# Fabri000/Maze-Solving-Agent-Gymnasium

Hardware: AMD Instinct MI355X
Metric: env steps/sec (whole node) + DQN win-rate, 40x40 r-prim mazes (higher is better)
Workload: dtype int32

## Files before the change

include/mazerl.h:

```cpp
#ifndef MAZERL_H
#define MAZERL_H
#include <stdint.h>

#ifdef __cplusplus
extern "C" {
#endif

#define MZ_OK 0
#define MZ_EINVAL (-1)
#define MZ_EINVAL_SHAPE (-2)
#define MZ_EHIP (-3)
#define MZ_ENOMEM (-4)
#define MZ_EALIGN (-5)

#define MZ_MAX_DIM 127
#define MZ_BANK_MAX_DIMS 64
#define MZ_MAX_CANDIDATES 64
#define MZ_WINDOW 15
#define MZ_WINDOW_BITS 675
#define MZ_WINDOW_WORDS 22

#define MZ_ALGO_RPRIM 0
#define MZ_ALGO_DFS 1
#define MZ_ALGO_PRIMKILL 2
// ... 58 lines not shown
int mz_generate_state(mz_handle* h, int32_t env, int32_t dim, int32_t algo, uint32_t* state_host,
                      void* stream);

int mz_reset_all(mz_handle* h, const mz_step_out* out, void* stream);
int mz_reset_list(mz_handle* h, const int32_t* idx_dev, const int32_t* count_dev,
                  int32_t max_count, int32_t regen_won, uint64_t seed, uint32_t epoch,
                  const mz_step_out* out, void* stream);

int mz_reset_done(mz_handle* h, int32_t regen_won, uint64_t seed, uint32_t epoch,
                  const mz_step_out* out, void* stream);

int mz_step(mz_handle* h, const int32_t* actions_dev, const mz_step_out* out, void* stream);

#define MZ_STEP_COUNT_ZEROED 1
#define MZ_STEP_AUTORESET 2
int mz_step_ex(mz_handle* h, const int32_t* actions_dev, const mz_step_out* out, int32_t flags,
               void* stream);

int mz_step_act(mz_handle* h, const float* eps_dev, float eps_all, const int64_t* greedy_dev,
                uint64_t seed, uint64_t counter, int32_t* actions_out_dev, const mz_step_out* out,
                int32_t flags, void* stream);

int mz_direction_mask(mz_handle* h, int32_t probs, float* out4_dev, void* stream);

int mz_act(mz_handle* h, const float* eps_dev, float eps_all, const int64_t* greedy_dev,
           uint64_t seed, uint64_t counter, int32_t* actions_dev, void* stream);

int mz_expand_window(const uint32_t* bits_dev, float* out_dev, int32_t n, void* stream);

int mz_bank_create(mz_handle* h, int32_t slots, int32_t dim, uint32_t algo_mask);
// ... 226 lines not shown
```

maze-solving-agent-gymnasium_amd/csrc/mz_api.hip:

```cpp
#include <algorithm>
#include <cmath>
#include <cstdarg>
#include <cstdio>
#include <cstdlib>
#include <cstring>
#include <string>
#include <vector>

#include "../../include/mazerl.h"
#include "mz_common.h"
#include "mz_learner.h"
#include "mz_mcclendon.h"

struct MzHostFallback {
  int cap = 0, gstride = 0;
  uint8_t *grid_h = nullptr, *grid_d = nullptr;
  int32_t *info_h = nullptr, *info_d = nullptr;
  double *prod_h = nullptr, *prod_d = nullptr;
  int32_t *ok_h = nullptr, *ok_d = nullptr;
  int32_t* count_h = nullptr;
  int* count_d = nullptr;
  int32_t* map = nullptr;
};

// ... 30 lines not shown
};

struct mz_handle {
  mz_config cfg;
  MzDev d;
  std::vector<void*> allocs;
  uint8_t* staging = nullptr;
  size_t staging_bytes = 0;
  MzBankStore bank;
  MzCandStore gen;
  int* sel_stats = nullptr;
  int dbg = 0;
  std::vector<void*> host_allocs;
  MzCompact scr{};
  int scr_cap = 0;
};

namespace {

thread_local std::string g_err;

int fail(int code, const char* fmt, ...) {
  char buf[512];
  va_list ap;
  va_start(ap, fmt);
  vsnprintf(buf, sizeof buf, fmt, ap);
  va_end(ap);
  g_err = buf;
  return code;
}
// ... 34 lines not shown
  MzOut m;
  std::memset(&m, 0, sizeof m);
  if (!o) return m;
  m.reward = o->reward; m.reward64 = o->reward64; m.terminated = o->terminated;
  m.truncated = o->truncated; m.pos = o->pos; m.best_dir = o->best_dir; m.obs6 = o->obs6;
  m.window_bits = o->window_bits; m.window = o->window; m.done_idx = o->done_idx;
  m.done_count = o->done_count;
  return m;
}

int check_out(const mz_step_out* o) {
  if (o && o->window && (reinterpret_cast<uintptr_t>(o->window) & 15u))
    return fail(MZ_EALIGN, "window output must be 16-byte aligned");
  if (o && o->done_idx && !o->done_count) return fail(MZ_EINVAL, "done_idx needs done_count");
  return MZ_OK;
}

int check_dim(const mz_handle* h, int dim) {
  if (dim < 5 || dim > h->cfg.max_dim)
    return fail(MZ_EINVAL_SHAPE, "maze dim %d outside [5, max_dim=%d]", dim, h->cfg.max_dim);
  if ((dim & 1) == 0)
    return fail(MZ_EINVAL_SHAPE, "even maze dim %d (reference gen_maze raises IndexError, "
                "lib/maze_generation.py:197-203)", dim);
  if (h->cfg.enrich && !h->cfg.toroidal && dim < 15)
    return fail(MZ_EINVAL_SHAPE, "euclidean window needs dim >= 15 (extract_submaze, "
                "lib/maze_handler.py:18-45)");
  return MZ_OK;
}

template <typename T>
// ... 310 lines not shown

int mz_reset_done(mz_handle* h, int32_t regen_won, uint64_t seed, uint32_t epoch,
                  const mz_step_out* out, void* stream) {
  if (!h) return fail(MZ_EINVAL, "null handle");
  int rc = check_out(out);
  if (rc) return rc;
  DeviceGuard g(h->cfg.device);
  MZ_HIP(mz_launch_reset_done(h->d, regen_won ? 1 : 0, seed, epoch, to_dev(out),
                              static_cast<hipStream_t>(stream)));
  return MZ_OK;
}

int mz_step_ex(mz_handle* h, const int32_t* actions_dev, const mz_step_out* out, int32_t flags,
               void* stream) {
  if (!h || !actions_dev) return fail(MZ_EINVAL, "bad arguments");
  if (flags & ~(MZ_STEP_COUNT_ZEROED | MZ_STEP_AUTORESET)) return fail(MZ_EINVAL, "flags %d", flags);
  int rc = check_out(out);
  if (rc) return rc;
  DeviceGuard g(h->cfg.device);
  hipStream_t s = static_cast<hipStream_t>(stream);
  if (out && out->done_count && !(flags & MZ_STEP_COUNT_ZEROED))
    MZ_HIP(hipMemsetAsync(out->done_count, 0, sizeof(int32_t), s));
  MZ_HIP(mz_launch_step(h->d, actions_dev, nullptr, (flags & MZ_STEP_AUTORESET) != 0, to_dev(out), s));
  return MZ_OK;
}

int mz_step(mz_handle* h, const int32_t* actions_dev, const mz_step_out* out, void* stream) {
  return mz_step_ex(h, actions_dev, out, 0, stream);
}

int mz_step_act(mz_handle* h, const float* eps_dev, float eps_all, const int64_t* greedy_dev,
                uint64_t seed, uint64_t counter, int32_t* actions_out_dev, const mz_step_out* out,
                int32_t flags, void* stream) {
  if (!h) return fail(MZ_EINVAL, "null handle");
  if (flags & ~(MZ_STEP_COUNT_ZEROED | MZ_STEP_AUTORESET)) return fail(MZ_EINVAL, "flags %d", flags);
  int rc = check_out(out);
  if (rc) return rc;
  DeviceGuard g(h->cfg.device);
  hipStream_t s = static_cast<hipStream_t>(stream);
  if (out && out->done_count && !(flags & MZ_STEP_COUNT_ZEROED))
    MZ_HIP(hipMemsetAsync(out->done_count, 0, sizeof(int32_t), s));
  MzAct ap{eps_dev, eps_all, greedy_dev, seed, counter, actions_out_dev};
  MZ_HIP(mz_launch_step(h->d, nullptr, &ap, (flags & MZ_STEP_AUTORESET) != 0, to_dev(out), s));
  return MZ_OK;
}

int mz_direction_mask(mz_handle* h, int32_t probs, float* out4_dev, void* stream) {
  if (!h || !out4_dev) return fail(MZ_EINVAL, "bad arguments");
  if (reinterpret_cast<uintptr_t>(out4_dev) & 15u) return fail(MZ_EALIGN, "out4 must be 16-B aligned");
  DeviceGuard g(h->cfg.device);
  MZ_HIP(mz_launch_mask(h->d, probs, out4_dev, static_cast<hipStream_t>(stream)));
  return MZ_OK;
}

int mz_act(mz_handle* h, const float* eps_dev, float eps_all, const int64_t* greedy_dev,
           uint64_t seed, uint64_t counter, int32_t* actions_dev, void* stream) {
  if (!h || !actions_dev) return fail(MZ_EINVAL, "bad arguments");
  DeviceGuard g(h->cfg.device);
// ... 513 lines not shown
  bool same_bank = hdr[SH_BK_K] == (uint32_t)b.K && hdr[SH_BK_NA] == (uint32_t)b.nA &&
                   hdr[SH_BK_ND] == (uint32_t)b.nD && hdr[SH_BK_AMASK] == b.amask;
  for (int i = 0; same_bank && i < b.nD; ++i) same_bank = dims[i] == (uint8_t)b.dims[i];
  if (!same_bank)
    return fail(MZ_EINVAL, "env state has a maze bank of %u slots x %u algorithms x %u sizes "
                "(mask %u); this handle's is %d x %d x %d (mask %u)", hdr[SH_BK_K], hdr[SH_BK_NA],
                hdr[SH_BK_ND], hdr[SH_BK_AMASK], b.K, b.nA, b.nD, b.amask);
  if (bytes < state_size(h)) return fail(MZ_EINVAL, "state buffer of %llu bytes, %zu needed",
                                         (unsigned long long)bytes, state_size(h));
  const uint8_t* src = static_cast<const uint8_t*>(src_dev);
  size_t off = MZ_STATE_HEADER_BYTES;
  for (const Section& sec : state_sections(h)) {
    MZ_HIP(hipMemcpyAsync(sec.p, src + off, sec.bytes, hipMemcpyDeviceToDevice, s));
    off += (sec.bytes + 255) & ~(size_t)255;
  }
  if (b.K) {
    b.epoch[0] = hdr[SH_BK_EPOCH0];
    b.epoch[1] = hdr[SH_BK_EPOCH1];
  }
  return mz_bank_use(h, (int32_t)hdr[SH_BK_ACTIVE]);
}

int mz_maze_metrics(mz_handle* h, const int32_t* env_ids_dev, int32_t n, double* out_dev,
                    void* stream) {
  if (!h || !out_dev) return fail(MZ_EINVAL, "bad arguments");
  if (h->d.toroidal) return fail(MZ_EINVAL, "maze metrics are defined for euclidean mazes");
  if (!env_ids_dev) n = h->d.B;
  if (n < 0 || n > h->d.B) return fail(MZ_EINVAL, "n out of range");
  DeviceGuard g(h->cfg.device);
  MZ_HIP(mz_launch_metrics(h->d, env_ids_dev, n, out_dev, static_cast<hipStream_t>(stream)));
// ... 555 lines not shown
```

maze-solving-agent-gymnasium_amd/csrc/mz_common.h:

```cpp
#pragma once
#include <hip/hip_runtime.h>
#include <stdint.h>

#define MZ_CELL_D_MASK 0x1FFFu
#define MZ_CELL_CODE_SHIFT 13
#define MZ_CELL_OPEN (1u << 16)
#define MZ_CELL_NB_SHIFT 17
#define MZ_CELL_CNT_SHIFT 21
#define MZ_CELL_TAG_SHIFT 29
#define MZ_CELL_STATIC ((1u << MZ_CELL_CNT_SHIFT) - 1u)
#define MZ_STW_TAG_SHIFT 24

__host__ __device__ inline int mz_cell_count(uint32_t w, uint32_t tag) {
  return (w >> MZ_CELL_TAG_SHIFT) == tag ? (int)((w >> MZ_CELL_CNT_SHIFT) & 0xFFu) : 0;
}
#define MZ_TICKET_PYERR 8

struct MzDev {
  int B, P, toroidal, enrich;
  int NS, PW;
  uint32_t* cells;
  uint32_t* planes;
  uint32_t* meta0;
  uint32_t* meta1;
  uint32_t* posw;
  uint32_t* stw;
// ... 37 lines not shown
};

struct MzOut {
  float* reward;
  double* reward64;
  uint8_t* terminated;
  uint8_t* truncated;
  int32_t* pos;
  int32_t* best_dir;
  float* obs6;
  uint32_t* window_bits;
  float* window;
  int32_t* done_idx;
  int32_t* done_count;
  int window_nt;
};
#define MZ_WINDOW_NT_BYTES (256ull << 20)

__host__ __device__ inline int mz_dr(int a) { return a == 0 ? 1 : (a == 1 ? -1 : 0); }
__host__ __device__ inline int mz_dc(int a) { return a == 2 ? 1 : (a == 3 ? -1 : 0); }
__host__ __device__ inline int mz_wrap(int v, int n) { v %= n; return v < 0 ? v + n : v; }
__host__ __device__ inline int mz_wrapn(int v, int n) {
  while (v < 0) v += n;
  while (v >= n) v -= n;
  return v;
}

__host__ __device__ inline void mz_philox(uint64_t key, uint64_t ctr_hi, uint64_t ctr_lo,
                                          uint32_t out[4]) {
  uint32_t c0 = (uint32_t)ctr_lo, c1 = (uint32_t)(ctr_lo >> 32), c2 = (uint32_t)ctr_hi,
// ... 59 lines not shown
```

maze-solving-agent-gymnasium_amd/csrc/mz_env.hip:

```cpp
#include "mz_common.h"
#include "mz_kernels.h"
#include "mz_build.inc.h"

#include "../../include/mazerl.h"

#define WAVE 64
#ifndef MZ_IPW
#define MZ_IPW 16
#endif
#define IPW MZ_IPW
#ifndef MZ_SPW
#define MZ_SPW 1
#endif
#ifndef MZ_PROBE
#define MZ_PROBE 0
#endif
__host__ __device__ constexpr int cat_words(int ipw) { return ipw * 675 / 32 + 2; }

namespace {

__device__ inline uint32_t wrap_colmask(int col, int C0, int N) {
  uint32_t m = 0;
  for (int j = mz_wrapn(col - C0, N); j < 15; j += N) m |= 1u << j;
  return m;
}

template <bool TOR>
__device__ inline int win_geo(int r, int c, int N) {
  int R0, C0;
  if (!TOR) { R0 = mz_win_start(r, N); C0 = mz_win_start(c, N); }
// ... 74 lines not shown
__device__ inline void write_obs6(float* o6, int r, int c, int gr, int gc, int br, int bc, int N) {
  if (ENRICH) {
    const double n = (double)N;
    o6[0] = (float)__ddiv_rn((double)r, n);
    o6[1] = (float)__ddiv_rn((double)c, n);
    o6[2] = (float)__ddiv_rn((double)gr, n);
    o6[3] = (float)__ddiv_rn((double)gc, n);
  } else {
    o6[0] = (float)r; o6[1] = (float)c; o6[2] = (float)gr; o6[3] = (float)gc;
  }
  o6[4] = (float)br;
  o6[5] = (float)bc;
}

typedef __attribute__((ext_vector_type(4))) unsigned int mz_u32x4;
template <int POL = 16>
__device__ inline void store_window_f32(const uint32_t* cat, float* out, int nb, int lane) {
  const int nfl = nb * 675;
  const int nq = nfl >> 2;
  const auto rsrc = __builtin_amdgcn_make_buffer_rsrc(out, 0, nfl * 4, 0x00020000);
  auto put = [&](int q, uint32_t word) {
    const uint32_t nib = (word >> ((q & 7) * 4)) & 0xFu;
    float4 v;
    v.x = (float)(nib & 1u);
    v.y = (float)((nib >> 1) & 1u);
    v.z = (float)((nib >> 2) & 1u);
    v.w = (float)((nib >> 3) & 1u);
    if (POL == 0) reinterpret_cast<float4*>(out)[q] = v;
    else __builtin_amdgcn_raw_buffer_store_b128(__builtin_bit_cast(mz_u32x4, v), rsrc, q * 16, 0, POL);
  };
  int q = lane;
  for (; q + 7 * WAVE < nq; q += 8 * WAVE) {
    uint32_t w[8];
#pragma unroll
    for (int u = 0; u < 8; ++u) w[u] = (MZ_PROBE & 32) ? (uint32_t)q * 0x9E3779B9u : cat[(q >> 3) + 8 * u];
#pragma unroll
    for (int u = 0; u < 8; ++u) put(q + u * WAVE, w[u]);
  }
  for (; q < nq; q += WAVE) put(q, cat[q >> 3]);
  for (int f = (nq << 2) + lane; f < nfl; f += WAVE) out[f] = (float)((cat[f >> 5] >> (f & 31)) & 1u);
}

__device__ inline void store_window_bits(const uint32_t* cat, uint32_t* wb, int nb, int lane) {
  for (int k = lane; k < nb * MZ_WINDOW_WORDS; k += WAVE) {
    const int j = k / MZ_WINDOW_WORDS, w = k - j * MZ_WINDOW_WORDS;
// ... 109 lines not shown
  else if (trans) {
    tr = r + mz_dr(a); tc = c + mz_dc(a);
    bool inb = true;
    if (TOR) { tr = mz_wrapn(tr, N); tc = mz_wrapn(tc, N); }
    else inb = 0 < tr && tr < N - 1 && 0 < tc && tc < N - 1;
    mv = inb && ((cw >> (MZ_CELL_NB_SHIFT + a)) & 1u);
    if (!mv) { tr = r; tc = c; }
  }

  const uint32_t tag = (sw >> MZ_STW_TAG_SHIFT) & 7u;
  uint32_t ncw = 0u;
  if ((mv || rst) && !(MZ_PROBE & 256)) ncw = d.cells[es * d.P * d.P + (size_t)tr * d.P + tc];
  const int cnt = rst ? 0 : mz_cell_count(ncw, tag);
  uint2 wr[win_it(IPWT)];
  int geo = 0;
  if (ENRICH) {
    if (live) geo = win_geo<TOR>(tr, tc, N);
#pragma unroll
    for (int it = 0; it < win_it(IPWT); ++it) {
      const int j = it * (WAVE / 16) + (lane >> 4), i = lane & 15;
      const int g = __shfl(geo, j);
      wr[it] = make_uint2(0u, 0u);
      if (j < nb && i < 15 && !(MZ_PROBE & 256)) wr[it] = *mz_strip_row(d, (size_t)(e0 + j), geo_st(g), geo_row<TOR>(g, i));
    }
  }
  __syncthreads();

  double rew = 0.0;
  bool term = false, trunc = false, done = false;
  int vr = -1, vc = -1;
  uint32_t ntag = tag;
  if (rst) {
    r = sr; c = sc; cw = ncw; nm = 0; la = 0; steps = 0; inv = 0;
    ntag = (tag + 1u) & 7u;
    vr = sr; vc = sc;
  } else if (trans) {
    if (mv) {
      if (cnt == 0) {
// ... 15 lines not shown
      rew = pen[256 + inv];
    }
    steps = min(steps + 1, 65535);
    trunc = steps > maxs;
    if (trunc) rew = -1.0;
    done = term || trunc;
  }

  if (ENRICH && !(MZ_PROBE & 2)) {
    const int ps = (int)rst | ((vr + 1) << 8) | ((vc + 1) << 16);
    const int pg = gr | (gc << 8);
#pragma unroll
    for (int it = 0; it < win_it(IPWT); ++it) {
      const int j = it * (WAVE / 16) + (lane >> 4), i = lane & 15;
      const int s_ = __shfl(ps, j), g = __shfl(geo, j), gg = __shfl(pg, j);
      if (j < nb && i < 15) {
        uint32_t c0, c1, c2;
        win_row_bits<TOR>(wr[it], g, geo_row<TOR>(g, i), gg & 0xFF, (gg >> 8) & 0xFF,
                          ((s_ >> 8) & 0xFF) - 1, ((s_ >> 16) & 0xFF) - 1, s_ & 1, c0, c1, c2);
        const int base = j * 675 + i * 15;
        if (MZ_PROBE & 512) {
          if ((c0 ^ (c1 << 1) ^ (c2 << 2)) == ((uint32_t)(lane * 77 + it) & 0x1FFFFu)) cat[0] = 1u;
        } else {
          cat_put(cat, base, c0);
          cat_put(cat, base + 225, c1);
          cat_put(cat, base + 450, c2);
        }
      }
    }
  }

  if ((rst || trans) && !(MZ_PROBE & 64)) {
    d.posw[e] = (uint32_t)r | ((uint32_t)c << 8) | ((uint32_t)nm << 16) | ((uint32_t)la << 18) |
                ((uint32_t)done << 20);
    d.stw[e] = (uint32_t)steps | ((uint32_t)inv << 16) | (ntag << MZ_STW_TAG_SHIFT);
    d.curw[e] = cw;
    d.last_term[e] = term;
    if (mv) {
      if (ENRICH && vr >= 0) mark_visited<TOR>(d, es, tr, tc, N);
      d.cells[es * d.P * d.P + (size_t)tr * d.P + tc] =
          (ncw & MZ_CELL_STATIC) | ((uint32_t)min(cnt + 1, 255) << MZ_CELL_CNT_SHIFT) |
          (tag << MZ_CELL_TAG_SHIFT);
    }
  }
  if (live && !(MZ_PROBE & 8)) {
    if (ACT && ap.act_out) ap.act_out[e] = rst ? -1 : araw;
    int br, bc;
    best_dir(r, c, cw, N, TOR, br, bc);
    if (o.reward) o.reward[e] = (float)rew;
    if (o.reward64) o.reward64[e] = rew;
    if (o.terminated) o.terminated[e] = term;
    if (o.truncated) o.truncated[e] = trunc;
    if (o.pos) { o.pos[2 * es] = r; o.pos[2 * es + 1] = c; }
    if (o.best_dir) { o.best_dir[2 * es] = br; o.best_dir[2 * es + 1] = bc; }
    if (o.obs6) write_obs6<ENRICH>(o.obs6 + 6 * es, r, c, gr, gc, br, bc, N);
  }
  if (ENRICH) {
    __syncthreads();
    if (o.window_bits) store_window_bits(cat, o.window_bits + (size_t)e0 * MZ_WINDOW_WORDS, nb, lane);
    if (o.window && !(MZ_PROBE & 16)) {
      if (o.window_nt) store_window_f32<2>(cat, o.window + (size_t)e0 * 675, nb, lane);
      else store_window_f32<16>(cat, o.window + (size_t)e0 * 675, nb, lane);
    }
  }

  if (AR && !(MZ_PROBE & 4)) {
    unsigned long long bal = __ballot(rst);
    const int sp = sr | (sc << 8) | ((int)ntag << 16) | (N << 19);
    while (bal) {
      const int j = __ffsll((long long)bal) - 1;
      bal &= bal - 1;
      const int q = __shfl(sp, j);
      const size_t ej = (size_t)(e0 + j);
      const int Nj = (q >> 19) & 0xFF;
      reset_visited(d, ej, Nj, q & 0xFF, (q >> 8) & 0xFF, TOR, lane);
      if (((q >> 16) & 7) == 0) clear_counts(d, ej, Nj);
    }
// ... 615 lines not shown
    if (!d.last_term[e] || dim == 0) continue;
    mz_build_one(d, e, d.toroidal, true, d.algo[e], seed + (uint64_t)e + ((uint64_t)epoch << 32),
                 dim, nullptr, 0, 0, 0, 0, lds);
    __syncthreads();
  }
}

__global__ void k_mask(MzDev d, int probs, float* out4) {
  const int e = blockIdx.x * blockDim.x + threadIdx.x;
  if (e >= d.B) return;
  float m[4];
  dir_mask(d.posw[e], d.curw[e], d.toroidal, probs, m);
  reinterpret_cast<float4*>(out4)[e] = make_float4(m[0], m[1], m[2], m[3]);
}

constexpr int GR_BLOCK = MZ_GR_BLOCK;
__device__ inline bool greedy_needed(const MzAct& ap, int e) {
  uint32_t u[4];
  act_u(ap, e, u);
  return act_greedy(u, ap.eps ? ap.eps[e] : ap.eps_all);
}

__global__ __launch_bounds__(GR_BLOCK) void k_greedy_count(MzAct ap, int n, int32_t* blk) {
  const int e = blockIdx.x * GR_BLOCK + threadIdx.x;
  const int c = __syncthreads_count(e < n && greedy_needed(ap, e));
  if (threadIdx.x == 0) blk[blockIdx.x] = c;
}

__global__ __launch_bounds__(GR_BLOCK) void k_greedy_list(MzAct ap, int n,
                                                          const int32_t* __restrict__ blk,
// ... 154 lines not shown
}

hipError_t mz_launch_step(const MzDev& d, const int32_t* act, const MzAct* ap, bool autoreset,
                          const MzOut& o0, hipStream_t s) {
  MzAct a{};
  if (ap) a = *ap;
  MzOut o = o0;
  o.window_nt = o.window && (size_t)d.B * 675 * sizeof(float) > MZ_WINDOW_NT_BYTES;
  if (d.toroidal) {
    if (d.enrich) launch_step_te<true, true>(d, act, a, ap != nullptr, autoreset, o, s);
    else launch_step_te<true, false>(d, act, a, ap != nullptr, autoreset, o, s);
  } else {
    if (d.enrich) launch_step_te<false, true>(d, act, a, ap != nullptr, autoreset, o, s);
    else launch_step_te<false, false>(d, act, a, ap != nullptr, autoreset, o, s);
  }
  return hipGetLastError();
}

hipError_t mz_launch_reset_list(const MzDev& d, const int32_t* idx, int32_t* count,
                                int32_t n_static, const MzOut& o, hipStream_t s) {
  if (n_static <= 0) return hipSuccess;
  const int blocks = n_static < 1024 ? n_static : 1024;
#define MZ_RL(T, E) \
  hipLaunchKernelGGL((k_reset_list<T, E>), dim3(blocks), dim3(WAVE), 0, s, d, idx, count, n_static, o)
  if (d.toroidal) { if (d.enrich) MZ_RL(true, true); else MZ_RL(true, false); }
  else { if (d.enrich) MZ_RL(false, true); else MZ_RL(false, false); }
#undef MZ_RL
  hipError_t e = hipGetLastError();
  if (e == hipSuccess && count) e = hipMemsetAsync(count, 0, sizeof(int32_t), s);
  return e;
// ... 209 lines not shown
```

maze-solving-agent-gymnasium_amd/csrc/mz_kernels.h:

```cpp
#pragma once
#include "mz_common.h"
#include "mz_screen.h"

size_t mz_build_lds_size(int P);
hipError_t mz_launch_build(const MzDev& d, const int32_t* env_ids, int32_t n, bool generate,
                           const uint8_t* algo_list, int32_t algo_all, int32_t dim, uint64_t seed,
                           const uint8_t* grids, const int32_t* start_goal, int pymode,
                           uint32_t* py_state, hipStream_t s);
hipError_t mz_launch_regen(const MzDev& d, const int32_t* idx, const int32_t* count,
                           int32_t n_static, uint64_t seed, uint32_t epoch, hipStream_t s);
hipError_t mz_launch_step(const MzDev& d, const int32_t* act, const MzAct* ap, bool autoreset,
                          const MzOut& o, hipStream_t s);
hipError_t mz_launch_reset_list(const MzDev& d, const int32_t* idx, int32_t* count,
                                int32_t n_static, const MzOut& o, hipStream_t s);
hipError_t mz_launch_meta(const MzDev& d, int32_t* out, hipStream_t s);
hipError_t mz_launch_returns(const double* rew, int ld, const int32_t* rows, const int32_t* lens,
                             int n, double gamma, float* out, int ldo, hipStream_t s);
hipError_t mz_launch_reset_done(const MzDev& d, int regen, uint64_t seed, uint32_t epoch,
                                const MzOut& o, hipStream_t s);
hipError_t mz_launch_mask(const MzDev& d, int probs, float* out4, hipStream_t s);
hipError_t mz_launch_act(const MzDev& d, const MzAct& ap, hipStream_t s);
hipError_t mz_launch_greedy_rows(const MzAct& ap, int n, int32_t* blk, int32_t* rows,
                                 int32_t* count, int32_t* count_host, hipStream_t s);
hipError_t mz_launch_expand(const uint32_t* bits, float* out, int n, hipStream_t s);
hipError_t mz_launch_qfront(const uint32_t* bits, const float* obs6, const int32_t* rows,
                            const int32_t* count, int n, const float* w, const float* b,
                            float drop_p, uint64_t seed, uint64_t counter, uint16_t* out, int ld,
// ... 36 lines not shown
```

maze-solving-agent-gymnasium_amd/mazerl/_native.py:

```python
import ctypes as C
import os

from . import _build

c_i32p = C.POINTER(C.c_int32)


class Config(C.Structure):
    _fields_ = [("num_envs", C.c_int32), ("max_dim", C.c_int32), ("toroidal", C.c_int32),
                ("enrich", C.c_int32), ("device", C.c_int32), ("reserved", C.c_int32 * 7)]


class StepOut(C.Structure):
    _fields_ = [("reward", C.c_void_p), ("reward64", C.c_void_p), ("terminated", C.c_void_p),
                ("truncated", C.c_void_p), ("pos", C.c_void_p), ("best_dir", C.c_void_p),
                ("obs6", C.c_void_p), ("window_bits", C.c_void_p), ("window", C.c_void_p),
                ("done_idx", C.c_void_p), ("done_count", C.c_void_p)]


class EnvInfo(C.Structure):
    _fields_ = [(k, C.c_int32) for k in ("n", "start_r", "start_c", "goal_r", "goal_c",
                                         "max_steps", "r", "c", "steps", "invalid_streak",
                                         "nmoves", "last_action", "done")]


MZ_STEP_COUNT_ZEROED = 1
MZ_STEP_AUTORESET = 2
MZ_RNG_PHILOX, MZ_RNG_CPYTHON = 0, 1
MZ_ERRORS = {-1: ValueError, -2: ValueError, -3: RuntimeError, -4: MemoryError, -5: ValueError}

EXPORTS = ["mz_last_error", "mz_device_count", "mz_create", "mz_destroy", "mz_load_mazes",
           "mz_generate", "mz_generate_ex", "mz_generate_state", "mz_reset_all", "mz_reset_list", "mz_reset_done", "mz_step", "mz_step_ex", "mz_direction_mask",
           "mz_act", "mz_step_act", "mz_expand_window", "mz_set_algorithm", "mz_query", "mz_get_grid",
           "mz_difficulty", "mz_maze_complexity", "mz_maze_metrics", "mz_difficulty_batch", "mz_get_meta", "mz_discounted_returns", "mz_q_front",
           "mz_bank_create", "mz_bank_create_dims", "mz_bank_create_ex", "mz_bank_fill", "mz_bank_use",
           "mz_bank_slot_grid", "mz_generate_best", "mz_select_stats", "mz_select_stats_ex",
           "mz_set_debug", "mz_screen_batch", "mz_set_regen_dims",
           "mz_bank_consumed", "mz_state_bytes", "mz_state_save", "mz_state_load",
           "mz_stem_forward", "mz_stem_backward", "mz_stem_backward_ex", "mz_stem_workspace_floats", "mz_adamw_flat",
           "mz_pair_surrogate", "mz_leaky_relu_bf16", "mz_colsum_f32",
           "mz_replay_gather", "mz_host_alloc", "mz_host_free", "mz_q_front_rows", "mz_greedy_rows",
           "mz_trainer_tick", "mz_greedy_scatter", "mz_head_bf16", "mz_replay_push",
           "mz_replay_sample_idx", "mz_q_loss", "mz_q_loss_backward", "mz_head_loss",
           "mz_head_loss_backward", "mz_head_loss_workspace_floats",
           "mz_head_loss_backward_workspace_floats", "mz_adamw_groups",
           "mz_ppo_act", "mz_ppo_scan", "mz_ppo_finish", "mz_ppo_head_loss", "mz_qact_prepare", "mz_qact",
           "mz_qact_workspace_floats", "mz_qtab_states", "mz_qtab_act", "mz_qtab_update",
           "mz_qtab_hash_act", "mz_qtab_hash_update", "mz_qtab_hash_rehash", "mz_qtab_hash_lookup"]
# ... 23 lines not shown
    L.mz_load_mazes.argtypes = [vp, vp, C.c_int32, vp, vp, C.c_int32, vp]
    L.mz_generate.argtypes = [vp, vp, C.c_int32, vp, C.c_int32, C.c_int32, C.c_uint64, vp]
    L.mz_generate_ex.argtypes = [vp, vp, C.c_int32, vp, C.c_int32, C.c_int32, C.c_uint64,
                                 C.c_int32, vp]
    L.mz_generate_state.argtypes = [vp, C.c_int32, C.c_int32, C.c_int32, vp, vp]
    L.mz_reset_all.argtypes = [vp, C.POINTER(StepOut), vp]
    L.mz_reset_list.argtypes = [vp, vp, vp, C.c_int32, C.c_int32, C.c_uint64, C.c_uint32,
                                C.POINTER(StepOut), vp]
    L.mz_reset_done.argtypes = [vp, C.c_int32, C.c_uint64, C.c_uint32, C.POINTER(StepOut), vp]
    L.mz_step.argtypes = [vp, vp, C.POINTER(StepOut), vp]
    L.mz_step_ex.argtypes = [vp, vp, C.POINTER(StepOut), C.c_int32, vp]
    L.mz_direction_mask.argtypes = [vp, C.c_int32, vp, vp]
    L.mz_act.argtypes = [vp, vp, C.c_float, vp, C.c_uint64, C.c_uint64, vp, vp]
    L.mz_step_act.argtypes = [vp, vp, C.c_float, vp, C.c_uint64, C.c_uint64, vp,
                              C.POINTER(StepOut), C.c_int32, vp]
    L.mz_expand_window.argtypes = [vp, vp, C.c_int32, vp]
    L.mz_set_algorithm.argtypes = [vp, vp, C.c_int32, vp]
    L.mz_query.argtypes = [vp, C.c_int32, C.POINTER(EnvInfo)]
    L.mz_get_grid.argtypes = [vp, C.c_int32, vp]
    L.mz_get_meta.argtypes = [vp, vp, vp]
    L.mz_discounted_returns.argtypes = [vp, C.c_int32, vp, vp, C.c_int32, C.c_double, vp,
                                        C.c_int32, vp]
    L.mz_difficulty.argtypes = [vp] + [C.c_int32] * 6 + [C.POINTER(C.c_double)]
    L.mz_maze_complexity.argtypes = [vp] + [C.c_int32] * 6 + [C.POINTER(C.c_double)] * 2
    L.mz_maze_metrics.argtypes = [vp, vp, C.c_int32, vp, vp]
    L.mz_difficulty_batch.argtypes = [vp, vp, C.c_int32, vp, vp, vp]
    L.mz_bank_create.argtypes = [vp, C.c_int32, C.c_int32, C.c_uint32]
    L.mz_bank_create_dims.argtypes = [vp, C.c_int32, vp, C.c_int32, C.c_uint32]
    L.mz_bank_create_ex.argtypes = [vp, C.c_int32, vp, C.c_int32, C.c_uint32, C.c_int32]
    L.mz_bank_fill.argtypes = [vp, C.c_int32, C.c_uint64, vp]
# ... 90 lines not shown
```

maze-solving-agent-gymnasium_amd/mazerl/vector_env.py:

```python
import torch

from . import _native as N

ALGOS = {"r-prim": 0, "dfs": 1, "prim&kill": 2}


def _ptr(t):
    return None if t is None else t.data_ptr()


def bank_seed(env_seed):
    return (0xBA4C0000 + (int(env_seed) - 0x5EED0000) * 0x9E3779B97F4A7C15) & 0xFFFFFFFFFFFFFFFF


class VectorMazeEnv:
    def __init__(self, num_envs, maze_dim, toroidal=False, enrich=True, device=None,
                 max_dim=None, algorithm="r-prim", seed=0x5EED0000, generate=True,
                 window=True, window_bits=True, reward64=False, pos=True, done_list=True,
                 host_scalars=False, candidates=1):
        if not torch.cuda.is_available():
            raise RuntimeError("VectorMazeEnv needs a HIP GPU (libmazerl.so has no CPU path)")
        self.lib = N.load()
        self.device = torch.device(device if device is not None else f"cuda:{torch.cuda.current_device()}")
        self.num_envs = int(num_envs)
        self.maze_dim = int(maze_dim)
        self.max_dim = int(max_dim or maze_dim)
        self.toroidal, self.enrich = bool(toroidal), bool(enrich)
        cfg = N.Config(num_envs=self.num_envs, max_dim=self.max_dim, toroidal=int(toroidal),
                       enrich=int(enrich), device=self.device.index or 0)
        h = N.C.c_void_p()
        N.check(self.lib.mz_create(N.C.byref(cfg), N.C.byref(h)))
        self._h = h
        B, dev = self.num_envs, self.device
        kw = dict(device=dev)
# ... 15 lines not shown
        self.done_idx = torch.zeros(B, dtype=torch.int32, **kw)
        self.done_count = torch.zeros(1, dtype=torch.int32, **kw)
        dp = self._dev_ptr
        self._out = N.StepOut(
            reward=dp(self.reward), reward64=dp(self.reward64), terminated=dp(self.terminated),
            truncated=dp(self.truncated), pos=dp(self.pos), best_dir=dp(self.best_dir),
            obs6=_ptr(self.obs6), window_bits=_ptr(self.window_bits), window=_ptr(self.window),
            done_idx=_ptr(self.done_idx) if done_list else None,
            done_count=_ptr(self.done_count) if done_list else None)
        self.seed = int(seed)
        self.epoch = 0
        self._bank = None
        self.algos_in_use = set()
        self._count_zero = True
        self._regen_dims = None
        if generate:
            self.generate(algorithm=algorithm, candidates=candidates)
            self.reset()

    def _stream(self):
        return torch.cuda.current_stream(self.device).cuda_stream

    def _alloc_host(self, B, reward64, pos):
        import numpy as np
        fields = [("actions", np.int32, (B,)), ("reward", np.float32, (B,)),
                  ("reward64", np.float64, (B,)) if reward64 else None,
                  ("terminated", np.uint8, (B,)), ("truncated", np.uint8, (B,)),
                  ("pos", np.int32, (B, 2)) if pos else None,
                  ("best_dir", np.int32, (B, 2)) if pos else None]
        offs, total = [], 0
# ... 271 lines not shown
        self.algos_in_use = set(sd.get("algos_in_use", ()))
        self.set_regen_dims(sd.get("regen_dims"))
        if bank is not None:
            self._bank.update(swap=int(bank["swap"]), calls=int(bank["calls"]),
                              cur=int(bank["cur"]), seed=int(bank["seed"]), ready=[None, None])
            self._bank["side"].wait_stream(torch.cuda.current_stream(self.device))
        self._host_sync()

    def reset_done_list(self, regen_won=False, seed=None):
        self.reset_list(self.done_idx, self.done_count, regen_won=regen_won, seed=seed)

    def step_host(self, action, env=0):
        if self._host is None:
            raise RuntimeError("step_host needs VectorMazeEnv(host_scalars=True)")
        self.actions[env] = int(action)
        N.check(self.lib.mz_step_ex(self._h, self._dev_ptr(self.actions), N.C.byref(self._out), 0,
                                    self._stream()))
        self._count_zero = False
        torch.cuda.current_stream(self.device).synchronize()

    def sync(self):
        torch.cuda.current_stream(self.device).synchronize()

    def step(self, actions, autoreset=False):
        a = actions if (actions.dtype == torch.int32 and actions.device == self.device) else \
            actions.to(device=self.device, dtype=torch.int32)
        a = a.contiguous()
        flags = N.MZ_STEP_AUTORESET if autoreset else 0
        N.check(self.lib.mz_step_ex(self._h, self._dev_ptr(a), N.C.byref(self._out), flags,
                                    self._stream()))
        self._count_zero = False
        self._host_sync()
        return self.obs(), self.reward, self.truncated, self.terminated, {}

    def step_act(self, eps=1.0, greedy=None, seed=0, counter=0, actions_out=None, autoreset=False):
        out = self.actions if actions_out is None else actions_out
        out_p = self._dev_ptr(out)
        eps_t = eps if torch.is_tensor(eps) else None
        g = None if greedy is None else greedy.to(dtype=torch.int64).contiguous()
        flags = N.MZ_STEP_COUNT_ZEROED if self._count_zero else 0
        if autoreset:
            flags |= N.MZ_STEP_AUTORESET
        N.check(self.lib.mz_step_act(self._h, _ptr(eps_t), float(eps) if eps_t is None else 0.0,
                                     _ptr(g), seed & 0xFFFFFFFFFFFFFFFF,
                                     counter & 0xFFFFFFFFFFFFFFFF, out_p,
                                     N.C.byref(self._out), flags, self._stream()))
        self._count_zero = False
        self._host_sync()
        return self.obs(), self.reward, self.truncated, self.terminated, {}

    def obs(self):
        o = {"obs6": self.obs6}
        if self.pos is not None:
            o["agent"], o["best dir"] = self.pos, self.best_dir
        if self.window is not None:
            o["window"] = self.window
        if self.window_bits is not None:
            o["window_bits"] = self.window_bits
        return o

    def direction_mask(self, probs=False, out=None):
        out = out if out is not None else torch.empty(self.num_envs, 4, dtype=torch.float32, device=self.device)
        N.check(self.lib.mz_direction_mask(self._h, int(bool(probs)), out.data_ptr(), self._stream()))
        return out
# ... 42 lines not shown
```

Baseline: 1.998 billion.

## Add delta window output: skip rewriting unchanged float windows between steps

Adds an opt-out flag that lets the step kernel skip reloading strip rows and rewriting the 675-float window for environments whose window origin did not change since the last step into the same buffer. Only the visited-cell entry is patched when the agent moves onto a new cell. Validity is tracked through a new posw bit, the last output pointer on the host, and an invalidation kernel run on state load. The aim is to cut global memory write bandwidth for the window output. The cost is extra per-element branching for partially kept float4 groups, plus a correctness risk if the caller modifies the window buffer between steps.

Result: no change. 2.012 billion, median of 6 (+0.7%).

```diff
diff --git a/include/mazerl.h b/include/mazerl.h
--- a/include/mazerl.h
+++ b/include/mazerl.h
@@ -96,6 +96,8 @@
 
 #define MZ_STEP_COUNT_ZEROED 1
 #define MZ_STEP_AUTORESET 2
+#define MZ_STEP_WINDOW_DELTA 4
+int mz_window_invalidate(mz_handle* h);
 int mz_step_ex(mz_handle* h, const int32_t* actions_dev, const mz_step_out* out, int32_t flags,
                void* stream);
 
diff --git a/maze-solving-agent-gymnasium_amd/csrc/mz_api.hip b/maze-solving-agent-gymnasium_amd/csrc/mz_api.hip
--- a/maze-solving-agent-gymnasium_amd/csrc/mz_api.hip
+++ b/maze-solving-agent-gymnasium_amd/csrc/mz_api.hip
@@ -68,6 +68,7 @@
   std::vector<void*> host_allocs;
   MzCompact scr{};
   int scr_cap = 0;
+  const float* last_window = nullptr;
 };
 
 namespace {
@@ -132,6 +133,13 @@
     return fail(MZ_EALIGN, "window output must be 16-byte aligned");
   if (o && o->done_idx && !o->done_count) return fail(MZ_EINVAL, "done_idx needs done_count");
   return MZ_OK;
+}
+
+MzOut step_out(mz_handle* h, const mz_step_out* out, int32_t flags) {
+  MzOut m = to_dev(out);
+  m.window_delta = (flags & MZ_STEP_WINDOW_DELTA) && m.window && m.window == h->last_window;
+  h->last_window = m.window;
+  return m;
 }
 
 int check_dim(const mz_handle* h, int dim) {
@@ -472,14 +480,15 @@
 int mz_step_ex(mz_handle* h, const int32_t* actions_dev, const mz_step_out* out, int32_t flags,
                void* stream) {
   if (!h || !actions_dev) return fail(MZ_EINVAL, "bad arguments");
-  if (flags & ~(MZ_STEP_COUNT_ZEROED | MZ_STEP_AUTORESET)) return fail(MZ_EINVAL, "flags %d", flags);
+  if (flags & ~(MZ_STEP_COUNT_ZEROED | MZ_STEP_AUTORESET | MZ_STEP_WINDOW_DELTA)) return fail(MZ_EINVAL, "flags %d", flags);
   int rc = check_out(out);
   if (rc) return rc;
   DeviceGuard g(h->cfg.device);
   hipStream_t s = static_cast<hipStream_t>(stream);
   if (out && out->done_count && !(flags & MZ_STEP_COUNT_ZEROED))
     MZ_HIP(hipMemsetAsync(out->done_count, 0, sizeof(int32_t), s));
-  MZ_HIP(mz_launch_step(h->d, actions_dev, nullptr, (flags & MZ_STEP_AUTORESET) != 0, to_dev(out), s));
+  MZ_HIP(mz_launch_step(h->d, actions_dev, nullptr, (flags & MZ_STEP_AUTORESET) != 0,
+                        step_out(h, out, flags), s));
   return MZ_OK;
 }
 
@@ -491,7 +500,7 @@
                 uint64_t seed, uint64_t counter, int32_t* actions_out_dev, const mz_step_out* out,
                 int32_t flags, void* stream) {
   if (!h) return fail(MZ_EINVAL, "null handle");
-  if (flags & ~(MZ_STEP_COUNT_ZEROED | MZ_STEP_AUTORESET)) return fail(MZ_EINVAL, "flags %d", flags);
+  if (flags & ~(MZ_STEP_COUNT_ZEROED | MZ_STEP_AUTORESET | MZ_STEP_WINDOW_DELTA)) return fail(MZ_EINVAL, "flags %d", flags);
   int rc = check_out(out);
   if (rc) return rc;
   DeviceGuard g(h->cfg.device);
@@ -499,7 +508,14 @@
   if (out && out->done_count && !(flags & MZ_STEP_COUNT_ZEROED))
     MZ_HIP(hipMemsetAsync(out->done_count, 0, sizeof(int32_t), s));
   MzAct ap{eps_dev, eps_all, greedy_dev, seed, counter, actions_out_dev};
-  MZ_HIP(mz_launch_step(h->d, nullptr, &ap, (flags & MZ_STEP_AUTORESET) != 0, to_dev(out), s));
+  MZ_HIP(mz_launch_step(h->d, nullptr, &ap, (flags & MZ_STEP_AUTORESET) != 0,
+                        step_out(h, out, flags), s));
+  return MZ_OK;
+}
+
+int mz_window_invalidate(mz_handle* h) {
+  if (!h) return fail(MZ_EINVAL, "null handle");
+  h->last_window = nullptr;
   return MZ_OK;
 }
 
@@ -1043,6 +1059,8 @@
     MZ_HIP(hipMemcpyAsync(sec.p, src + off, sec.bytes, hipMemcpyDeviceToDevice, s));
     off += (sec.bytes + 255) & ~(size_t)255;
   }
+  MZ_HIP(mz_launch_window_invalid(d, s));
+  h->last_window = nullptr;
   if (b.K) {
     b.epoch[0] = hdr[SH_BK_EPOCH0];
     b.epoch[1] = hdr[SH_BK_EPOCH1];
diff --git a/maze-solving-agent-gymnasium_amd/csrc/mz_common.h b/maze-solving-agent-gymnasium_amd/csrc/mz_common.h
--- a/maze-solving-agent-gymnasium_amd/csrc/mz_common.h
+++ b/maze-solving-agent-gymnasium_amd/csrc/mz_common.h
@@ -10,6 +10,7 @@
 #define MZ_CELL_TAG_SHIFT 29
 #define MZ_CELL_STATIC ((1u << MZ_CELL_CNT_SHIFT) - 1u)
 #define MZ_STW_TAG_SHIFT 24
+#define MZ_POSW_WINVALID (1u << 21)
 
 __host__ __device__ inline int mz_cell_count(uint32_t w, uint32_t tag) {
   return (w >> MZ_CELL_TAG_SHIFT) == tag ? (int)((w >> MZ_CELL_CNT_SHIFT) & 0xFFu) : 0;
@@ -77,6 +78,7 @@
   int32_t* done_idx;
   int32_t* done_count;
   int window_nt;
+  int window_delta;
 };
 #define MZ_WINDOW_NT_BYTES (256ull << 20)
 
diff --git a/maze-solving-agent-gymnasium_amd/csrc/mz_env.hip b/maze-solving-agent-gymnasium_amd/csrc/mz_env.hip
--- a/maze-solving-agent-gymnasium_amd/csrc/mz_env.hip
+++ b/maze-solving-agent-gymnasium_amd/csrc/mz_env.hip
@@ -14,6 +14,9 @@
 #endif
 #ifndef MZ_PROBE
 #define MZ_PROBE 0
+#endif
+#ifndef MZ_DELTA_VARIANT
+#define MZ_DELTA_VARIANT 0
 #endif
 __host__ __device__ constexpr int cat_words(int ipw) { return ipw * 675 / 32 + 2; }
 
@@ -118,8 +121,9 @@
 }
 
 typedef __attribute__((ext_vector_type(4))) unsigned int mz_u32x4;
-template <int POL = 16>
-__device__ inline void store_window_f32(const uint32_t* cat, float* out, int nb, int lane) {
+template <int POL>
+__device__ __forceinline__ void store_window_f32(const uint32_t* cat, float* out, int nb, int lane,
+                                                 uint32_t kept) {
   const int nfl = nb * 675;
   const int nq = nfl >> 2;
   const auto rsrc = __builtin_amdgcn_make_buffer_rsrc(out, 0, nfl * 4, 0x00020000);
@@ -133,6 +137,31 @@
     if (POL == 0) reinterpret_cast<float4*>(out)[q] = v;
     else __builtin_amdgcn_raw_buffer_store_b128(__builtin_bit_cast(mz_u32x4, v), rsrc, q * 16, 0, POL);
   };
+  if (kept) {
+    auto putk = [&](int q, uint32_t word) {
+      const int f0 = q << 2, j0 = f0 / 675, n0 = (j0 + 1) * 675 - f0;
+      const bool k0 = (kept >> j0) & 1u, k1 = n0 < 4 ? (bool)((kept >> (j0 + 1)) & 1u) : k0;
+      if (!k0 && !k1) put(q, word);
+      else if (k0 != k1) {
+        const uint32_t nib = (word >> ((q & 7) * 4)) & 0xFu;
+#pragma unroll
+        for (int t = 0; t < 4; ++t)
+          if (t < n0 ? !k0 : !k1) out[f0 + t] = (float)((nib >> t) & 1u);
+      }
+    };
+    int q = lane;
+    for (; q + 7 * WAVE < nq; q += 8 * WAVE) {
+      uint32_t w[8];
+#pragma unroll
+      for (int u = 0; u < 8; ++u) w[u] = cat[(q >> 3) + 8 * u];
+#pragma unroll
+      for (int u = 0; u < 8; ++u) putk(q + u * WAVE, w[u]);
+    }
+    for (; q < nq; q += WAVE) putk(q, cat[q >> 3]);
+    for (int f = (nq << 2) + lane; f < nfl; f += WAVE)
+      if (!((kept >> (f / 675)) & 1u)) out[f] = (float)((cat[f >> 5] >> (f & 31)) & 1u);
+    return;
+  }
   int q = lane;
   for (; q + 7 * WAVE < nq; q += 8 * WAVE) {
     uint32_t w[8];
@@ -272,14 +301,22 @@
   const int cnt = rst ? 0 : mz_cell_count(ncw, tag);
   uint2 wr[win_it(IPWT)];
   int geo = 0;
+  uint32_t kept = 0u, skip = 0u;
+  bool keep = false;
   if (ENRICH) {
     if (live) geo = win_geo<TOR>(tr, tc, N);
+    if (o.window_delta && MZ_DELTA_VARIANT != 2) {
+      keep = live && !rst && (pw & MZ_POSW_WINVALID) && win_geo<TOR>(r, c, N) == geo;
+      kept = (uint32_t)__ballot(keep);
+      if (!o.window_bits && MZ_DELTA_VARIANT != 1) skip = kept;
+    }
 #pragma unroll
     for (int it = 0; it < win_it(IPWT); ++it) {
       const int j = it * (WAVE / 16) + (lane >> 4), i = lane & 15;
       const int g = __shfl(geo, j);
       wr[it] = make_uint2(0u, 0u);
-      if (j < nb && i < 15 && !(MZ_PROBE & 256)) wr[it] = *mz_strip_row(d, (size_t)(e0 + j), geo_st(g), geo_row<TOR>(g, i));
+      if (j < nb && i < 15 && !((skip >> j) & 1u) && !(MZ_PROBE & 256))
+        wr[it] = *mz_strip_row(d, (size_t)(e0 + j), geo_st(g), geo_row<TOR>(g, i));
     }
   }
   __syncthreads();
@@ -325,7 +362,7 @@
     for (int it = 0; it < win_it(IPWT); ++it) {
       const int j = it * (WAVE / 16) + (lane >> 4), i = lane & 15;
       const int s_ = __shfl(ps, j), g = __shfl(geo, j), gg = __shfl(pg, j);
-      if (j < nb && i < 15) {
+      if (j < nb && i < 15 && !((skip >> j) & 1u)) {
         uint32_t c0, c1, c2;
         win_row_bits<TOR>(wr[it], g, geo_row<TOR>(g, i), gg & 0xFF, (gg >> 8) & 0xFF,
                           ((s_ >> 8) & 0xFF) - 1, ((s_ >> 16) & 0xFF) - 1, s_ & 1, c0, c1, c2);
@@ -343,7 +380,7 @@
 
   if ((rst || trans) && !(MZ_PROBE & 64)) {
     d.posw[e] = (uint32_t)r | ((uint32_t)c << 8) | ((uint32_t)nm << 16) | ((uint32_t)la << 18) |
-                ((uint32_t)done << 20);
+                ((uint32_t)done << 20) | ((ENRICH && o.window) ? MZ_POSW_WINVALID : 0u);
     d.stw[e] = (uint32_t)steps | ((uint32_t)inv << 16) | (ntag << MZ_STW_TAG_SHIFT);
     d.curw[e] = cw;
     d.last_term[e] = term;
@@ -370,8 +407,14 @@
     __syncthreads();
     if (o.window_bits) store_window_bits(cat, o.window_bits + (size_t)e0 * MZ_WINDOW_WORDS, nb, lane);
     if (o.window && !(MZ_PROBE & 16)) {
-      if (o.window_nt) store_window_f32<2>(cat, o.window + (size_t)e0 * 675, nb, lane);
-      else store_window_f32<16>(cat, o.window + (size_t)e0 * 675, nb, lane);
+      if (keep && mv && cnt == 0) {
+        const int wi = TOR ? mz_wrapn(tr - (geo & 0x7F), N) : tr - (geo & 0x7F);
+        const int C0 = MZ_STRIP_STRIDE * geo_st(geo) + ((geo >> 10) & 31);
+        const int wj = TOR ? mz_wrapn(tc - C0, N) : tc - C0;
+        if ((unsigned)wi < 15u && (unsigned)wj < 15u) o.window[es * 675 + 450 + wi * 15 + wj] = 0.0f;
+      }
+      if (o.window_nt) store_window_f32<2>(cat, o.window + (size_t)e0 * 675, nb, lane, kept);
+      else store_window_f32<16>(cat, o.window + (size_t)e0 * 675, nb, lane, kept);
     }
   }
 
@@ -1017,6 +1060,11 @@
   reinterpret_cast<float4*>(out4)[e] = make_float4(m[0], m[1], m[2], m[3]);
 }
 
+__global__ void k_window_invalid(MzDev d) {
+  const int e = blockIdx.x * blockDim.x + threadIdx.x;
+  if (e < d.B) d.posw[e] &= ~MZ_POSW_WINVALID;
+}
+
 constexpr int GR_BLOCK = MZ_GR_BLOCK;
 __device__ inline bool greedy_needed(const MzAct& ap, int e) {
   uint32_t u[4];
@@ -1201,6 +1249,11 @@
     if (d.enrich) launch_step_te<false, true>(d, act, a, ap != nullptr, autoreset, o, s);
     else launch_step_te<false, false>(d, act, a, ap != nullptr, autoreset, o, s);
   }
+  return hipGetLastError();
+}
+
+hipError_t mz_launch_window_invalid(const MzDev& d, hipStream_t s) {
+  hipLaunchKernelGGL(k_window_invalid, dim3((d.B + 255) / 256), dim3(256), 0, s, d);
   return hipGetLastError();
 }
 
diff --git a/maze-solving-agent-gymnasium_amd/csrc/mz_kernels.h b/maze-solving-agent-gymnasium_amd/csrc/mz_kernels.h
--- a/maze-solving-agent-gymnasium_amd/csrc/mz_kernels.h
+++ b/maze-solving-agent-gymnasium_amd/csrc/mz_kernels.h
@@ -11,6 +11,7 @@
                            int32_t n_static, uint64_t seed, uint32_t epoch, hipStream_t s);
 hipError_t mz_launch_step(const MzDev& d, const int32_t* act, const MzAct* ap, bool autoreset,
                           const MzOut& o, hipStream_t s);
+hipError_t mz_launch_window_invalid(const MzDev& d, hipStream_t s);
 hipError_t mz_launch_reset_list(const MzDev& d, const int32_t* idx, int32_t* count,
                                 int32_t n_static, const MzOut& o, hipStream_t s);
 hipError_t mz_launch_meta(const MzDev& d, int32_t* out, hipStream_t s);
diff --git a/maze-solving-agent-gymnasium_amd/mazerl/_native.py b/maze-solving-agent-gymnasium_amd/mazerl/_native.py
--- a/maze-solving-agent-gymnasium_amd/mazerl/_native.py
+++ b/maze-solving-agent-gymnasium_amd/mazerl/_native.py
@@ -26,12 +26,13 @@
 
 MZ_STEP_COUNT_ZEROED = 1
 MZ_STEP_AUTORESET = 2
+MZ_STEP_WINDOW_DELTA = 4
 MZ_RNG_PHILOX, MZ_RNG_CPYTHON = 0, 1
 MZ_ERRORS = {-1: ValueError, -2: ValueError, -3: RuntimeError, -4: MemoryError, -5: ValueError}
 
 EXPORTS = ["mz_last_error", "mz_device_count", "mz_create", "mz_destroy", "mz_load_mazes",
            "mz_generate", "mz_generate_ex", "mz_generate_state", "mz_reset_all", "mz_reset_list", "mz_reset_done", "mz_step", "mz_step_ex", "mz_direction_mask",
-           "mz_act", "mz_step_act", "mz_expand_window", "mz_set_algorithm", "mz_query", "mz_get_grid",
+           "mz_act", "mz_step_act", "mz_window_invalidate", "mz_expand_window", "mz_set_algorithm", "mz_query", "mz_get_grid",
            "mz_difficulty", "mz_maze_complexity", "mz_maze_metrics", "mz_difficulty_batch", "mz_get_meta", "mz_discounted_returns", "mz_q_front",
            "mz_bank_create", "mz_bank_create_dims", "mz_bank_create_ex", "mz_bank_fill", "mz_bank_use",
            "mz_bank_slot_grid", "mz_generate_best", "mz_select_stats", "mz_select_stats_ex",
@@ -85,6 +86,8 @@
     L.mz_act.argtypes = [vp, vp, C.c_float, vp, C.c_uint64, C.c_uint64, vp, vp]
     L.mz_step_act.argtypes = [vp, vp, C.c_float, vp, C.c_uint64, C.c_uint64, vp,
                               C.POINTER(StepOut), C.c_int32, vp]
+    if hasattr(L, "mz_window_invalidate"):
+        L.mz_window_invalidate.argtypes = [vp]
     L.mz_expand_window.argtypes = [vp, vp, C.c_int32, vp]
     L.mz_set_algorithm.argtypes = [vp, vp, C.c_int32, vp]
     L.mz_query.argtypes = [vp, C.c_int32, C.POINTER(EnvInfo)]
diff --git a/maze-solving-agent-gymnasium_amd/mazerl/vector_env.py b/maze-solving-agent-gymnasium_amd/mazerl/vector_env.py
--- a/maze-solving-agent-gymnasium_amd/mazerl/vector_env.py
+++ b/maze-solving-agent-gymnasium_amd/mazerl/vector_env.py
@@ -1,3 +1,5 @@
+import os
+
 import torch
 
 from . import _native as N
@@ -17,7 +19,7 @@
     def __init__(self, num_envs, maze_dim, toroidal=False, enrich=True, device=None,
                  max_dim=None, algorithm="r-prim", seed=0x5EED0000, generate=True,
                  window=True, window_bits=True, reward64=False, pos=True, done_list=True,
-                 host_scalars=False, candidates=1):
+                 host_scalars=False, candidates=1, window_delta=None):
         if not torch.cuda.is_available():
             raise RuntimeError("VectorMazeEnv needs a HIP GPU (libmazerl.so has no CPU path)")
         self.lib = N.load()
@@ -63,6 +65,11 @@
         self.algos_in_use = set()
         self._count_zero = True
         self._regen_dims = None
+        if window_delta is None:
+            window_delta = os.environ.get("MAZERL_WINDOW_DELTA") != "0"
+        self._step_flags = N.MZ_STEP_WINDOW_DELTA if (
+            window_delta and self.window is not None
+            and hasattr(self.lib, "mz_window_invalidate")) else 0
         if generate:
             self.generate(algorithm=algorithm, candidates=candidates)
             self.reset()
@@ -364,8 +371,8 @@
         if self._host is None:
             raise RuntimeError("step_host needs VectorMazeEnv(host_scalars=True)")
         self.actions[env] = int(action)
-        N.check(self.lib.mz_step_ex(self._h, self._dev_ptr(self.actions), N.C.byref(self._out), 0,
-                                    self._stream()))
+        N.check(self.lib.mz_step_ex(self._h, self._dev_ptr(self.actions), N.C.byref(self._out),
+                                    self._step_flags, self._stream()))
         self._count_zero = False
         torch.cuda.current_stream(self.device).synchronize()
 
@@ -376,7 +383,7 @@
         a = actions if (actions.dtype == torch.int32 and actions.device == self.device) else \
             actions.to(device=self.device, dtype=torch.int32)
         a = a.contiguous()
-        flags = N.MZ_STEP_AUTORESET if autoreset else 0
+        flags = self._step_flags | (N.MZ_STEP_AUTORESET if autoreset else 0)
         N.check(self.lib.mz_step_ex(self._h, self._dev_ptr(a), N.C.byref(self._out), flags,
                                     self._stream()))
         self._count_zero = False
@@ -388,7 +395,7 @@
         out_p = self._dev_ptr(out)
         eps_t = eps if torch.is_tensor(eps) else None
         g = None if greedy is None else greedy.to(dtype=torch.int64).contiguous()
-        flags = N.MZ_STEP_COUNT_ZEROED if self._count_zero else 0
+        flags = self._step_flags | (N.MZ_STEP_COUNT_ZEROED if self._count_zero else 0)
         if autoreset:
             flags |= N.MZ_STEP_AUTORESET
         N.check(self.lib.mz_step_act(self._h, _ptr(eps_t), float(eps) if eps_t is None else 0.0,
@@ -398,6 +405,10 @@
         self._count_zero = False
         self._host_sync()
         return self.obs(), self.reward, self.truncated, self.terminated, {}
+
+    def invalidate_window(self):
+        if self._step_flags:
+            N.check(self.lib.mz_window_invalidate(self._h))
 
     def obs(self):
         o = {"obs6": self.obs6}
diff --git a/profiles/window_kept_share.py b/profiles/window_kept_share.py
--- /dev/null
+++ b/profiles/window_kept_share.py
@@ -0,0 +1,56 @@
+import argparse
+import json
+import os
+import sys
+
+import torch
+
+ROOT = os.path.dirname(os.path.dirname(os.path.abspath(__file__)))
+sys.path.insert(0, os.path.join(ROOT, "maze-solving-agent-gymnasium_amd"))
+import mazerl
+
+
+def win_start(p, n):
+    if n == 15:
+        return torch.zeros_like(p)
+    return torch.clamp(p - 7, 0, n - 15)
+
+
+def main():
+    ap = argparse.ArgumentParser()
+    ap.add_argument("--envs", type=int, default=65536)
+    ap.add_argument("--dim", type=int, default=81)
+    ap.add_argument("--warmup", type=int, default=100)
+    ap.add_argument("--steps", type=int, default=200)
+    a = ap.parse_args()
+    env = mazerl.VectorMazeEnv(a.envs, a.dim, enrich=True, algorithm="r-prim", seed=0x5EED0000,
+                               window=True, window_bits=False, pos=True, done_list=False)
+    for k in range(a.warmup):
+        env.step_act(eps=1.0, seed=0xBE7C4, counter=k, autoreset=True)
+    n = kept = patched = resets = moved = 0
+    ar = torch.arange(a.envs, device=env.device)
+    for k in range(a.warmup, a.warmup + a.steps):
+        p0 = env.pos.clone().long()
+        done = (env.terminated | env.truncated).bool()
+        w0 = env.window.clone()
+        env.step_act(eps=1.0, seed=0xBE7C4, counter=k, autoreset=True)
+        p1 = env.pos.long()
+        o0, o1 = win_start(p0, a.dim), win_start(p1, a.dim)
+        keep = ~done & (o0 == o1).all(1)
+        mv = (p0 != p1).any(1)
+        wi, wj = (p1 - o1)[:, 0], (p1 - o1)[:, 1]
+        first = w0[ar, 2, wi, wj] == 1.0
+        n += a.envs
+        kept += int(keep.sum())
+        patched += int((keep & mv & first).sum())
+        resets += int(done.sum())
+        moved += int((~done & mv).sum())
+    print(json.dumps({"envs": a.envs, "dim": a.dim, "warmup": a.warmup, "steps": a.steps,
+                      "instance_steps": n, "kept_share": kept / n, "patched_share": patched / n,
+                      "unchanged_share": (kept - patched) / n, "reset_share": resets / n,
+                      "moved_share": moved / n}))
+    env.close()
+
+
+if __name__ == "__main__":
+    main()
```
